# czbiohub-sf/shrimPy

Hardware: AMD Instinct MI355X
Metric: voxels/sec deskew+20-iter RL deconv, 2048×2048×512 f32; HBM GB/s vs peak (higher is better)
Workload: dtype f32

## Files before the change

shrimpy_amd/csrc/rl_fused_sep.hip:

```cpp

#include "common.hpp"
#include "correlate_common.hpp"

#ifndef LSR_FUSED_PZ
#error "compile with -DLSR_FUSED_PZ=<odd tap count along z>"
#endif

namespace {

using lsr::FusedArgs;

constexpr int kTX = lsr::kSepWideTileX;
constexpr int kWaves = 8;
constexpr int kThreads = 64 * kWaves;
constexpr int kBand = 8;
constexpr int kRing = 3;

constexpr int cdiv(int a, int b) { return (a + b - 1) / b; }

template <int PZ, int PYX, int RUN>
struct Geo {
  static constexpr int C = PYX / 2, CZ = PZ / 2;
  static constexpr int TY = 8 * RUN;
  static constexpr int WL = lsr::fused_window_halo(PYX);
  static constexpr int AR = TY + 4 * C;
  static constexpr int PA = kTX + 2 * WL;
  static constexpr int CH = PA / 4;
  static constexpr int NCH = AR * CH;
  static constexpr int SL = cdiv(NCH, kThreads);
  static constexpr int ASZ = cdiv(NCH, 64) * 64 * 4;
  static constexpr int NP = cdiv(4 + 2 * C, 4);
  static constexpr int G1 = (kTX + WL) / 4;
  static constexpr int PB1 = 4 * G1;
  static constexpr int NIT1 = AR * G1;
  static constexpr int XIT1 = cdiv(NIT1, kThreads);
  static constexpr int R1 = TY + 2 * C;
  static constexpr int RUN1 = cdiv(R1, 8);
  static constexpr int E = PB1 - kTX;
  static constexpr int NE = R1 * E;
  static constexpr int EP = cdiv(NE, kThreads);
  static constexpr int SH = WL - 2 * C;
  static constexpr int PR = 4 * (kTX / 4 - 1 + NP);
  static constexpr int RSZ = 4 + 8 * RUN1 * PR;
  static constexpr int NIT2 = R1 * (kTX / 4);
  static constexpr int XIT2 = cdiv(NIT2, kThreads);
  static constexpr int B1SZ = AR * PB1;
  static constexpr int B2SZ = R1 * kTX;
  static constexpr int OFF_B1 = kRing * ASZ;
  static constexpr int OFF_R = OFF_B1 + B1SZ;
  static constexpr int OFF_B2 = OFF_R + RSZ;
  static constexpr int OFF_DUMP = OFF_B2 + B2SZ;
  static constexpr int OFF_RNY = OFF_DUMP + 256;
  static constexpr int TOTAL = OFF_RNY + 32;
  static constexpr int NY = 2 * RUN1 + EP;
#ifdef LSR_FUSED_PROBE_NOXC
  static constexpr int NXC = 0;
#else
  static constexpr int NXC = 2 * RUN + 1;
#endif
  static_assert(TOTAL * 4 <= 160 * 1024, "LDS per workgroup");
  static_assert(PR == PB1, "B1 and R share a pitch");
  static_assert(2 * C <= WL && WL <= lsr::kSepOriginCol, "halo columns");
  static_assert(SL + 2 * (NY + NXC) <= 63, "vmcnt is a 6-bit counter");
  static_assert(OFF_B1 % 4 == 0 && OFF_R % 4 == 0 && OFF_B2 % 4 == 0, "16-byte aligned buffers");
};

typedef float f32x4 __attribute__((ext_vector_type(4)));
typedef float f32x2 __attribute__((ext_vector_type(2)));

__device__ __forceinline__ float fast_rcp(float d) {
  float r = __builtin_amdgcn_rcpf(d);
  return fmaf(fmaf(-d, r, 1.0f), r, r);
}
__device__ __forceinline__ f32x2 splat(float a) { return f32x2{a, a}; }
__device__ __forceinline__ f32x2 pk_fma(f32x2 a, f32x2 b, f32x2 c) { return __builtin_elementwise_fma(a, b, c); }
__device__ __forceinline__ f32x2 fast_rcp2(f32x2 d) {
  const f32x2 r = f32x2{__builtin_amdgcn_rcpf(d.x), __builtin_amdgcn_rcpf(d.y)};
  return pk_fma(pk_fma(-d, r, splat(1.0f)), r, r);
}
template <int PX, int NP>
__device__ __forceinline__ f32x4 xpass_item(const f32x4* src, const float (&wx)[PX]) {
  float w[4 * NP];
#pragma unroll
  for (int i = 0; i < NP; ++i) {
    const f32x4 v = src[i];
    w[4 * i] = v.x; w[4 * i + 1] = v.y; w[4 * i + 2] = v.z; w[4 * i + 3] = v.w;
  }
  f32x2 o01 = splat(wx[0]) * f32x2{w[0], w[1]};
  f32x2 o23 = splat(wx[0]) * f32x2{w[2], w[3]};
#pragma unroll
  for (int c = 1; c < PX; ++c) {
    o01 = pk_fma(splat(wx[c]), f32x2{w[c], w[c + 1]}, o01);
    o23 = pk_fma(splat(wx[c]), f32x2{w[c + 2], w[c + 3]}, o23);
  }
  return f32x4{o01.x, o01.y, o23.x, o23.y};
}

template <int IMM>
__device__ __forceinline__ void gload(float& dst, const float* sbase, int voff) {
  asm volatile("global_load_dword %0, %1, %2 offset:%3" : "+v"(dst) : "v"(voff), "s"(sbase), "n"(IMM) : "memory");
}
#ifndef LSR_FUSED_STORE_POLICY
#define LSR_FUSED_STORE_POLICY "nt"
#endif
#ifndef LSR_FUSED_GLDS_POLICY
#define LSR_FUSED_GLDS_POLICY ""
#endif
template <int IMM>
__device__ __forceinline__ void gstore(float* sbase, int voff, float v) {
  asm volatile("global_store_dword %0, %1, %2 offset:%3 " LSR_FUSED_STORE_POLICY
               :
               : "v"(voff), "v"(v), "s"(sbase), "n"(IMM)
               : "memory");
}
__device__ __forceinline__ void glds_x4(const float* sbase, int voff, unsigned lds_byte_addr) {
  asm volatile("s_mov_b32 m0, %2\n\ts_nop 0\n\tglobal_load_lds_dwordx4 %0, %1 " LSR_FUSED_GLDS_POLICY
               :
               : "v"(voff), "s"(sbase), "s"(lds_byte_addr)
               : "memory");
}
template <int N>
__device__ __forceinline__ void wait_vm() {
  asm volatile("s_waitcnt vmcnt(%0)" : : "n"(N) : "memory");
}
template <int K>
__device__ __forceinline__ void tie(float (&a)[K]) {
#pragma unroll
  for (int i = 0; i < K; ++i) asm volatile("" : "+v"(a[i]));
}
__device__ __forceinline__ void tie(float& a) { asm volatile("" : "+v"(a)); }
__device__ __forceinline__ void lds_barrier() {
  asm volatile("s_waitcnt lgkmcnt(0)" ::: "memory");
  __builtin_amdgcn_s_barrier();
  __builtin_amdgcn_sched_barrier(0);
}

template <int PZ, int PYX, int RUN, bool STATS>
__global__ __launch_bounds__(kThreads) void rl_fused_sep_kernel(FusedArgs p) {
  using T = Geo<PZ, PYX, RUN>;
  constexpr int C = T::C, CZ = T::CZ, TY = T::TY, RUN1 = T::RUN1, EP = T::EP;
  constexpr int NP = T::NP, NY = T::NY, NXC = T::NXC, SL = T::SL;
  __shared__ f32x4 smem4[T::TOTAL / 4];
  float* const smem = reinterpret_cast<float*>(smem4);
  f32x4* const B1_4 = smem4 + T::OFF_B1 / 4;
  const float* const B1 = smem + T::OFF_B1;
  float* const Rw = smem + T::OFF_R + 4;
  const f32x4* const R_4 = smem4 + T::OFF_R / 4 + 1;
  f32x4* const B2_4 = smem4 + T::OFF_B2 / 4;
  const float* const B2 = smem + T::OFF_B2;
  const unsigned lds_base =
      static_cast<unsigned>(reinterpret_cast<size_t>((__attribute__((address_space(3))) char*)smem4));

  const int tid = threadIdx.x;
  const int lane = tid & 63;
  const int wave = __builtin_amdgcn_readfirstlane(tid >> 6);

  auto xcd_contiguous = [](int b, int n) {
#ifdef LSR_FUSED_PLAIN_ORDER
    return b;
#endif
    const int per = n / 8, rem = n % 8;
    const int xcd = b % 8, idx = b / 8;
    return xcd * per + (xcd < rem ? xcd : rem) + idx;
  };
  const int Z = p.Z, Y = p.Y, X = p.X;
  int lin, zb, ze;
  if (static_cast<int>(blockIdx.x) < p.n_full) {
    lin = xcd_contiguous(blockIdx.x, p.n_full);
    zb = 0;
    ze = Z;
  } else {
    const int t = xcd_contiguous(blockIdx.x - p.n_full, gridDim.x - p.n_full);
    const int col = t / p.pieces;
    lin = p.n_full + col;
    zb = (t - col * p.pieces) * p.z_chunk;
    ze = min(zb + p.z_chunk, Z);
  }
  const int band = lin / (p.tiles_x * kBand);
  const int lb = lin - band * (p.tiles_x * kBand);
  const int band_h = min(kBand, p.tiles_y - band * kBand);
#if defined(LSR_FUSED_PLAIN_ORDER) && LSR_FUSED_PLAIN_ORDER == 2
  const int tx = lin % p.tiles_x;
  const int ty = lin / p.tiles_x;
  (void)lb; (void)band_h;
#else
  const int tx = lb / band_h;
  const int ty = band * kBand + (lb - tx * band_h);
#endif
  const int x0 = tx * kTX, y0 = ty * TY;
#ifdef LSR_FUSED_LAG
  if ((tx + ty) & 1) {
#pragma unroll
    for (int i = 0; i < LSR_FUSED_LAG; ++i) __builtin_amdgcn_s_sleep(127);
  }
#endif

  float tv0 = p.taps[lane], tv1 = p.taps[64 + (lane & 31)];
  auto load_taps = [&](int row, auto& w) {
#pragma unroll
    for (int i = 0; i < static_cast<int>(sizeof(w) / sizeof(float)); ++i) {
      const int f = row * 16 + i;
      w[i] = __int_as_float(__builtin_amdgcn_readlane(__float_as_int(f < 64 ? tv0 : tv1), f & 63));
    }
  };

  const float* const x_tile = p.x + (static_cast<int64_t>(y0 - 2 * C) * p.pitch + (x0 - T::WL));
  int s_voff[SL];
#pragma unroll
  for (int k = 0; k < SL; ++k) {
    const int e = min(tid + k * kThreads, T::NCH - 1);
    const int r = e / T::CH, c = e - r * T::CH;
    s_voff[k] = (r * p.pitch + 4 * c) * 4;
  }
  int a1_chunk[T::XIT1];
#pragma unroll
  for (int k = 0; k < T::XIT1; ++k) {
    const int i = min(tid + k * kThreads, T::NIT1 - 1);
    const int row = i / T::G1;
    a1_chunk[k] = i + row * (T::CH - T::G1);
  }
  const int r1_row0 = wave * RUN1;
  const int y1_col = r1_row0 * T::PB1 + lane;
  const int r_col = r1_row0 * T::PR + lane - T::SH;
  const bool interior = x0 - C >= 0 && x0 + kTX + C <= X && y0 - C >= 0 && y0 + TY + C <= Y;
  int e_b1[EP], e_voff[EP];
  int e_rc[EP];
#pragma unroll
  for (int e = 0; e < EP; ++e) {
    const int t = min(tid + e * kThreads, T::NE - 1);
    const int er = t / T::E, ec = t - er * T::E;
    e_b1[e] = er * T::PB1 + kTX + ec;
    e_rc[e] = (er << 16) | (kTX + ec);
    e_voff[e] = (er * p.y_pitch + kTX + ec) * 4;
  }
  const int y2_col = (wave * RUN) * kTX + lane;
  int xc_voff[RUN], o_voff[RUN], y_voff[RUN1];
#pragma unroll
  for (int m = 0; m < RUN; ++m) {
    xc_voff[m] = ((wave * RUN + m) * p.pitch + lane) * 4;
    o_voff[m] = ((wave * RUN + m) * p.out_pitch + lane) * 4;
  }
#pragma unroll
  for (int m = 0; m < RUN1; ++m) y_voff[m] = (min(r1_row0 + m, T::R1 - 1) * p.y_pitch + lane) * 4;
  float rnx[2];
#pragma unroll
  for (int cg = 0; cg < 2; ++cg) rnx[cg] = fast_rcp(p.nx[min(x0 + lane + 64 * cg, X - 1)]);
  float* const rny_lds = smem + T::OFF_RNY;
  if (tid < TY) rny_lds[tid] = fast_rcp(p.ny[min(y0 + tid, Y - 1)]);

  f32x2 acc1[PZ][RUN1], acc2[PZ][RUN];
  float acc1e[PZ][EP];
#pragma unroll
  for (int j = 0; j < PZ; ++j) {
#pragma unroll
    for (int i = 0; i < RUN1; ++i) acc1[j][i] = splat(0.0f);
#pragma unroll
    for (int i = 0; i < EP; ++i) acc1e[j][i] = 0.0f;
#pragma unroll
    for (int i = 0; i < RUN; ++i) acc2[j][i] = splat(0.0f);
  }
  float yv[2 * RUN1], ye[EP], xc[2 * RUN], nzv = 1.0f;
#pragma unroll
  for (int i = 0; i < 2 * RUN1; ++i) yv[i] = 0.0f;
#pragma unroll
  for (int i = 0; i < EP; ++i) ye[i] = 0.0f;
#pragma unroll
  for (int i = 0; i < 2 * RUN; ++i) xc[i] = 0.0f;
  const f32x2 rnx2 = f32x2{rnx[0], rnx[1]};
  f32x2 st_flux = splat(0.0f), st_total = splat(0.0f);
  float st_change = 0.0f;
  auto st_add = [&](f32x2 x_old, f32x2 xu, f32x2 v) {
    st_flux += xu;
    st_total += v;
    const f32x2 d = v - x_old;
    st_change += __builtin_fabsf(d.x);
    st_change += __builtin_fabsf(d.y);
  };
  __builtin_amdgcn_sched_barrier(0);

  auto clampz = [&](int z) { return min(max(z, 0), Z - 1); };
  auto issue_glds = [&](int plane, int slot) {
    const float* src = x_tile + static_cast<int64_t>(clampz(plane)) * p.plane;
    const unsigned dst = lds_base + (slot * T::ASZ + wave * 64 * 4) * 4;
#pragma unroll
    for (int k = 0; k < SL; ++k) {
      const bool live = wave * 64 + k * kThreads < T::NCH;
      glds_x4(src, s_voff[k], live ? dst + k * kThreads * 16 : lds_base + T::OFF_DUMP * 4);
    }
  };
  const float* const xc_tile = p.x + (static_cast<int64_t>(y0) * p.pitch + x0);
  const float* const y_tile = p.y + (static_cast<int64_t>(y0 - C) * p.y_pitch + (x0 + C - T::WL));
  float* const o_tile = p.out + (static_cast<int64_t>(y0) * p.out_pitch + x0);
  auto issue_xc = [&](int o) {
#ifdef LSR_FUSED_PROBE_NOXC
    return;
#endif
    const int oc = clampz(o);
    const float* base = xc_tile + static_cast<int64_t>(oc) * p.plane;
#pragma unroll
    for (int m = 0; m < RUN; ++m) {
      gload<0>(xc[m], base, xc_voff[m]);
      gload<256>(xc[RUN + m], base, xc_voff[m]);
    }
    gload<0>(nzv, p.nz + oc, 0);
  };
  auto issue_y = [&](int q) {
    const float* base = y_tile + static_cast<int64_t>(clampz(q)) * p.y_plane;
#pragma unroll
    for (int m = 0; m < RUN1; ++m) {
      gload<0>(yv[m], base, y_voff[m]);
      gload<256>(yv[RUN1 + m], base, y_voff[m]);
    }
#pragma unroll
    for (int e = 0; e < EP; ++e) gload<0>(ye[e], base, e_voff[e]);
  };

  const int q_lo = max(zb - CZ, 0), q_hi = min(ze - 1 + CZ, Z - 1);
  const int p_lo = max(q_lo - CZ, 0);
  const int p_hi = ze + 2 * CZ;

  int slot = 0;
  issue_glds(p_lo, 0);
  issue_xc(p_lo - 1 - 2 * CZ);
  issue_y(p_lo - CZ);
  issue_glds(p_lo + 1, 1);
  issue_xc(p_lo - 1 - 2 * CZ);
  issue_y(p_lo - CZ);
  wait_vm<SL + 2 * (NXC + NY)>();
  lds_barrier();

#ifdef LSR_FUSED_PROBE_TIME
  if (p.probe && tid == 0) p.probe[4 * blockIdx.x] = wall_clock64();
#endif
  for (int pz = p_lo; pz <= p_hi; ++pz) {
    asm volatile("" : "+v"(tv0), "+v"(tv1));
#ifdef LSR_FUSED_PROBE_TIME
    if (p.probe && tid == 0 && (pz == p_lo + 40 || pz == p_lo + 120))
      p.probe[4 * blockIdx.x + (pz == p_lo + 40 ? 1 : 2)] = wall_clock64();
#endif
    const int qr = pz - 1 - CZ;
    const int o = qr - CZ;
    const int q = pz - CZ;
    const bool x_live = pz < Z && pz <= q_hi + CZ;
    const bool r_live = qr >= q_lo && qr <= q_hi;
    const int slot2 = slot >= 1 ? slot - 1 : 2;

    issue_glds(pz + 2, slot2);
#ifdef LSR_FUSED_PROBE_NOCOMPUTE
    if (false) {
#else
    if (x_live) {
#endif
      float w1x[PYX];
      load_taps(0, w1x);
      const f32x4* A_4 = smem4 + slot * (T::ASZ / 4);
#pragma unroll
      for (int k = 0; k < T::XIT1; ++k)
        if (k + 1 < T::XIT1 || tid + k * kThreads < T::NIT1)
          B1_4[tid + k * kThreads] = xpass_item<PYX, NP>(A_4 + a1_chunk[k], w1x);
    } else {
#pragma unroll
      for (int k = 0; k < T::XIT1; ++k)
        if (k + 1 < T::XIT1 || tid + k * kThreads < T::NIT1) B1_4[tid + k * kThreads] = f32x4{0, 0, 0, 0};
    }
#ifdef LSR_FUSED_PROBE_NOCOMPUTE
    if (false) {
#else
    if (r_live) {
#endif
      float w2x[PYX];
      load_taps(3, w2x);
#pragma unroll
      for (int k = 0; k < T::XIT2; ++k) {
        const int j = tid + k * kThreads;
        if (k + 1 < T::XIT2 || j < T::NIT2)
          B2_4[j] = xpass_item<PYX, NP>(R_4 + (j + (j >> 5) * (T::PR / 4 - kTX / 4)), w2x);
      }
    } else {
#pragma unroll
      for (int k = 0; k < T::XIT2; ++k)
        if (k + 1 < T::XIT2 || tid + k * kThreads < T::NIT2) B2_4[tid + k * kThreads] = f32x4{0, 0, 0, 0};
    }
    lds_barrier();

    {
      float w2y[PYX], w2z[PZ];
      load_taps(4, w2y);
      load_taps(5, w2z);
      f32x2 pl[RUN];
#ifdef LSR_FUSED_PROBE_NOCOMPUTE
#pragma unroll
      for (int m = 0; m < RUN; ++m) pl[m] = splat(B2[y2_col + m]);
      if (false)
#endif
      {
        const float* colp = B2 + y2_col;
        f32x2 cv[RUN + 2 * C];
#pragma unroll
        for (int j = 0; j < RUN + 2 * C; ++j) cv[j] = f32x2{colp[j * kTX], colp[j * kTX + 64]};
#pragma unroll
        for (int m = 0; m < RUN; ++m) {
          f32x2 s2 = splat(w2y[0]) * cv[m];
#pragma unroll
          for (int b = 1; b < PYX; ++b) s2 = pk_fma(splat(w2y[b]), cv[m + b], s2);
          pl[m] = s2;
        }
      }
#pragma unroll
      for (int j = 0; j < PZ - 1; ++j)
#pragma unroll
        for (int i = 0; i < RUN; ++i) acc2[j][i] = pk_fma(splat(w2z[PZ - 1 - j]), pl[i], acc2[j + 1][i]);
#pragma unroll
      for (int i = 0; i < RUN; ++i) acc2[PZ - 1][i] = splat(w2z[0]) * pl[i];

      wait_vm<NY + SL>();
      tie(xc);
      tie(nzv);
#ifdef LSR_FUSED_PROBE_NOSTORE
      if (o >= zb && o < ze && nzv == 12345.678f) {
#else
      if (o >= zb && o < ze) {
#endif
        float* obase = o_tile + static_cast<int64_t>(o) * p.out_plane;
        const float rz = fast_rcp(nzv);
        if (!p.mask_out) {
#pragma unroll
          for (int m = 0; m < RUN; ++m) {
            const f32x2 xo = f32x2{xc[m], xc[RUN + m]};
            const f32x2 xu = xo * acc2[0][m];
            const f32x2 v = xu * (splat(rz * rny_lds[wave * RUN + m]) * rnx2);
            gstore<0>(obase, o_voff[m], v.x);
            gstore<256>(obase, o_voff[m], v.y);
            if constexpr (STATS) st_add(xo, xu, v);
          }
        } else {
          const bool ok0 = x0 + lane < X, ok1 = x0 + lane + 64 < X;
#pragma unroll
          for (int m = 0; m < RUN; ++m) {
            if (y0 + wave * RUN + m < Y) {
              const f32x2 xo = f32x2{xc[m], xc[RUN + m]};
              const f32x2 xu = xo * acc2[0][m];
              const f32x2 v = xu * (splat(rz * rny_lds[wave * RUN + m]) * rnx2);
              if (ok0) gstore<0>(obase, o_voff[m], v.x);
              if (ok1) gstore<256>(obase, o_voff[m], v.y);
              if constexpr (STATS) {
                st_add(xo, xu, v);
              }
            }
          }
        }
      }
      __builtin_amdgcn_sched_barrier(0);
      issue_xc(o + 1);
    }
    {
      float w1y[PYX], w1z[PZ];
      load_taps(1, w1y);
      load_taps(2, w1z);
      f32x2 pl[RUN1];
      float ple[EP];
#ifdef LSR_FUSED_PROBE_NOCOMPUTE
#pragma unroll
      for (int m = 0; m < RUN1; ++m) pl[m] = splat(B1[y1_col + m]);
      if (false)
#endif
      {
        const float* colp = B1 + y1_col;
        f32x2 cv[RUN1 + 2 * C];
#pragma unroll
        for (int j = 0; j < RUN1 + 2 * C; ++j) cv[j] = f32x2{colp[j * T::PB1], colp[j * T::PB1 + 64]};
#pragma unroll
        for (int m = 0; m < RUN1; ++m) {
          f32x2 s2 = splat(w1y[0]) * cv[m];
#pragma unroll
          for (int b = 1; b < PYX; ++b) s2 = pk_fma(splat(w1y[b]), cv[m + b], s2);
          pl[m] = s2;
        }
      }
#pragma unroll
      for (int e = 0; e < EP; ++e) {
        const float* colp = B1 + e_b1[e];
#ifdef LSR_FUSED_PROBE_NOCOMPUTE
        ple[e] = colp[0];
        continue;
#endif
        float s1 = w1y[0] * colp[0];
#pragma unroll
        for (int b = 1; b < PYX; ++b) s1 = fmaf(w1y[b], colp[b * T::PB1], s1);
        ple[e] = s1;
      }
#pragma unroll
      for (int j = 0; j < PZ - 1; ++j) {
#pragma unroll
        for (int i = 0; i < RUN1; ++i) acc1[j][i] = pk_fma(splat(w1z[PZ - 1 - j]), pl[i], acc1[j + 1][i]);
#pragma unroll
        for (int e = 0; e < EP; ++e) acc1e[j][e] = fmaf(w1z[PZ - 1 - j], ple[e], acc1e[j + 1][e]);
      }
#pragma unroll
      for (int i = 0; i < RUN1; ++i) acc1[PZ - 1][i] = splat(w1z[0]) * pl[i];
#pragma unroll
      for (int e = 0; e < EP; ++e) acc1e[PZ - 1][e] = w1z[0] * ple[e];

      wait_vm<SL + NXC>();
      tie(yv);
      tie(ye);
      const bool q_in = q >= q_lo && q <= q_hi;
      if (q_in && interior) {
#pragma unroll
        for (int m = 0; m < RUN1; ++m) {
          const f32x2 r = f32x2{yv[m], yv[RUN1 + m]} * fast_rcp2(acc1[0][m] + splat(p.eps));
          Rw[r_col + m * T::PR] = r.x;
          Rw[r_col + m * T::PR + 64] = r.y;
        }
#pragma unroll
        for (int e = 0; e < EP; ++e)
          if (e + 1 < EP || tid + e * kThreads < T::NE)
            Rw[e_b1[e] - T::SH] = ye[e] * fast_rcp(acc1e[0][e] + p.eps);
      } else {
        const int gx0 = x0 + lane + C - T::WL;
        const bool in0 = q_in && gx0 >= 0 && gx0 < X, in1 = q_in && gx0 + 64 >= 0 && gx0 + 64 < X;
#pragma unroll
        for (int m = 0; m < RUN1; ++m) {
          const int gy = y0 + r1_row0 + m - C;
          const bool row_in = gy >= 0 && gy < Y && r1_row0 + m < T::R1;
          const f32x2 r = f32x2{yv[m], yv[RUN1 + m]} * fast_rcp2(acc1[0][m] + splat(p.eps));
          Rw[r_col + m * T::PR] = (row_in && in0) ? r.x : 0.0f;
          Rw[r_col + m * T::PR + 64] = (row_in && in1) ? r.y : 0.0f;
        }
#pragma unroll
        for (int e = 0; e < EP; ++e) {
          if (e + 1 < EP || tid + e * kThreads < T::NE) {
            const int gy = y0 + (e_rc[e] >> 16) - C, gx = x0 + (e_rc[e] & 0xffff) + C - T::WL;
            const float r = ye[e] * fast_rcp(acc1e[0][e] + p.eps);
            Rw[e_b1[e] - T::SH] = (q_in && gy >= 0 && gy < Y && gx >= 0 && gx < X) ? r : 0.0f;
          }
        }
      }
      __builtin_amdgcn_sched_barrier(0);
      issue_y(q + 1);
    }
    wait_vm<SL + 2 * (NXC + NY)>();
    lds_barrier();
    slot = slot == 2 ? 0 : slot + 1;
  }
  asm volatile("s_waitcnt vmcnt(0)" ::: "memory");
  if constexpr (STATS) {
    lsr::keep_until_here(xc);
    lsr::keep_until_here(yv);
    lsr::keep_until_here(ye);
    lsr::keep_until_here(nzv);
    asm volatile("" : "+v"(st_flux), "+v"(st_total), "+v"(st_change));
    lsr::RlStats st;
    st.flux = st_flux.x + st_flux.y;
    st.change = st_change;
    st.total = st_total.x + st_total.y;
    lsr::rl_stats_flush<kWaves>(st, smem + T::OFF_B2, p.stats);
  }
#ifdef LSR_FUSED_PROBE_TIME
  if (p.probe && tid == 0) p.probe[4 * blockIdx.x + 3] = wall_clock64();
#endif
}

template <int PZ, int PYX>
bool launch_one(const FusedArgs& p, dim3 grid, hipStream_t s) {
  if constexpr (lsr::fused_compiled(PZ, PYX)) {
    constexpr int RUN = lsr::fused_run(PZ, PYX);
    if (p.stats != nullptr) hipLaunchKernelGGL((rl_fused_sep_kernel<PZ, PYX, RUN, true>), grid, dim3(kThreads), 0, s, p);
    else hipLaunchKernelGGL((rl_fused_sep_kernel<PZ, PYX, RUN, false>), grid, dim3(kThreads), 0, s, p);
    return true;
  } else {
    return false;
  }
}

}

namespace lsr {

#define LSR_CAT2(a, b) a##b
#define LSR_CAT(a, b) LSR_CAT2(a, b)
bool LSR_CAT(launch_fused_pz, LSR_FUSED_PZ)(int pyx, const FusedArgs& p, unsigned blocks, hipStream_t s) {
  constexpr int PZ = LSR_FUSED_PZ;
  const dim3 grid(blocks);
  switch (pyx) {
    case 3: return launch_one<PZ, 3>(p, grid, s);
    case 5: return launch_one<PZ, 5>(p, grid, s);
    case 7: return launch_one<PZ, 7>(p, grid, s);
    case 9: return launch_one<PZ, 9>(p, grid, s);
    case 11: return launch_one<PZ, 11>(p, grid, s);
    case 13: return launch_one<PZ, 13>(p, grid, s);
    case 15: return launch_one<PZ, 15>(p, grid, s);
    default: return false;
  }
}

}
```

Baseline: 40.46 billion.

## Keep delayed x planes in an LDS delay line instead of re-reading from HBM

```diff
diff --git a/shrimpy_amd/csrc/rl_fused_sep.hip b/shrimpy_amd/csrc/rl_fused_sep.hip
--- a/shrimpy_amd/csrc/rl_fused_sep.hip
+++ b/shrimpy_amd/csrc/rl_fused_sep.hip
@@ -14,9 +14,10 @@
 constexpr int kWaves = 8;
 constexpr int kThreads = 64 * kWaves;
 constexpr int kBand = 8;
-constexpr int kRing = 3;
+constexpr int kLdsFloats = 160 * 1024 / 4;
 
 constexpr int cdiv(int a, int b) { return (a + b - 1) / b; }
+constexpr int imin(int a, int b) { return a < b ? a : b; }
 
 template <int PZ, int PYX, int RUN>
 struct Geo {
@@ -46,23 +47,43 @@
   static constexpr int XIT2 = cdiv(NIT2, kThreads);
   static constexpr int B1SZ = AR * PB1;
   static constexpr int B2SZ = R1 * kTX;
-  static constexpr int OFF_B1 = kRing * ASZ;
+  static constexpr int D = PZ;
+  static constexpr int HXW = 8 * kTX * D;
+  static constexpr int FIXED = B1SZ + RSZ + B2SZ + 256 + 32;
+  static constexpr int hold_fit(int ring) {
+    return imin(RUN, (kLdsFloats - FIXED - ring * ASZ) / HXW);
+  }
+#ifdef LSR_FUSED_HOLD
+  static constexpr int HL = imin(LSR_FUSED_HOLD, hold_fit(2));
+#else
+  static constexpr int HL = hold_fit(3) > 0 ? hold_fit(3) : hold_fit(2);
+#endif
+#ifdef LSR_FUSED_RING
+  static constexpr int RING = LSR_FUSED_RING;
+#else
+  static constexpr int RING = HL <= hold_fit(3) ? 3 : 2;
+#endif
+  static constexpr int HOLD = 8 * HL;
+  static constexpr int OFF_B1 = RING * ASZ;
   static constexpr int OFF_R = OFF_B1 + B1SZ;
   static constexpr int OFF_B2 = OFF_R + RSZ;
   static constexpr int OFF_DUMP = OFF_B2 + B2SZ;
   static constexpr int OFF_RNY = OFF_DUMP + 256;
-  static constexpr int TOTAL = OFF_RNY + 32;
+  static constexpr int OFF_HX = OFF_RNY + 32;
+  static constexpr int TOTAL = OFF_HX + HL * HXW;
   static constexpr int NY = 2 * RUN1 + EP;
 #ifdef LSR_FUSED_PROBE_NOXC
   static constexpr int NXC = 0;
 #else
-  static constexpr int NXC = 2 * RUN + 1;
-#endif
+  static constexpr int NXC = 2 * (RUN - HL) + 1;
+#endif
+  static constexpr int VM_RING = (RING - 2) * SL + (RING - 1) * (NXC + NY);
   static_assert(TOTAL * 4 <= 160 * 1024, "LDS per workgroup");
   static_assert(PR == PB1, "B1 and R share a pitch");
   static_assert(2 * C <= WL && WL <= lsr::kSepOriginCol, "halo columns");
-  static_assert(SL + 2 * (NY + NXC) <= 63, "vmcnt is a 6-bit counter");
-  static_assert(OFF_B1 % 4 == 0 && OFF_R % 4 == 0 && OFF_B2 % 4 == 0, "16-byte aligned buffers");
+  static_assert(VM_RING <= 63 && SL + NY <= 63 && SL + NXC <= 63, "vmcnt is a 6-bit counter");
+  static_assert(OFF_B1 % 4 == 0 && OFF_R % 4 == 0 && OFF_B2 % 4 == 0 && OFF_HX % 4 == 0, "16-byte aligned buffers");
+  static_assert(0 <= HL && HL <= RUN && (RING == 3 || RING == 2), "delay line");
 };
 
 typedef float f32x4 __attribute__((ext_vector_type(4)));
@@ -139,7 +160,7 @@
 __global__ __launch_bounds__(kThreads) void rl_fused_sep_kernel(FusedArgs p) {
   using T = Geo<PZ, PYX, RUN>;
   constexpr int C = T::C, CZ = T::CZ, TY = T::TY, RUN1 = T::RUN1, EP = T::EP;
-  constexpr int NP = T::NP, NY = T::NY, NXC = T::NXC, SL = T::SL;
+  constexpr int NP = T::NP, NY = T::NY, NXC = T::NXC, SL = T::SL, HL = T::HL, RING = T::RING;
   __shared__ f32x4 smem4[T::TOTAL / 4];
   float* const smem = reinterpret_cast<float*>(smem4);
   f32x4* const B1_4 = smem4 + T::OFF_B1 / 4;
@@ -259,13 +280,15 @@
 #pragma unroll
     for (int i = 0; i < RUN; ++i) acc2[j][i] = splat(0.0f);
   }
-  float yv[2 * RUN1], ye[EP], xc[2 * RUN], nzv = 1.0f;
+  constexpr int NXR = RUN - HL;
+  constexpr int NXV = NXR > 0 ? 2 * NXR : 1;
+  float yv[2 * RUN1], ye[EP], xc[NXV], nzv = 1.0f;
 #pragma unroll
   for (int i = 0; i < 2 * RUN1; ++i) yv[i] = 0.0f;
 #pragma unroll
   for (int i = 0; i < EP; ++i) ye[i] = 0.0f;
 #pragma unroll
-  for (int i = 0; i < 2 * RUN; ++i) xc[i] = 0.0f;
+  for (int i = 0; i < NXV; ++i) xc[i] = 0.0f;
   const f32x2 rnx2 = f32x2{rnx[0], rnx[1]};
   f32x2 st_flux = splat(0.0f), st_total = splat(0.0f);
   float st_change = 0.0f;
@@ -298,9 +321,9 @@
     const int oc = clampz(o);
     const float* base = xc_tile + static_cast<int64_t>(oc) * p.plane;
 #pragma unroll
-    for (int m = 0; m < RUN; ++m) {
-      gload<0>(xc[m], base, xc_voff[m]);
-      gload<256>(xc[RUN + m], base, xc_voff[m]);
+    for (int m = HL; m < RUN; ++m) {
+      gload<0>(xc[m - HL], base, xc_voff[m]);
+      gload<256>(xc[NXR + m - HL], base, xc_voff[m]);
     }
     gload<0>(nzv, p.nz + oc, 0);
   };
@@ -320,13 +343,19 @@
   const int p_hi = ze + 2 * CZ;
 
   int slot = 0;
+  constexpr int HX_STEP = HL * kWaves * kTX;
+  int hx_i = T::OFF_HX + wave * kTX + lane;
+  int xa_i = (2 * C + wave * RUN) * T::PA + T::WL + lane;
+  if constexpr (HL > 0) asm volatile("" : "+v"(hx_i), "+v"(xa_i));
   issue_glds(p_lo, 0);
   issue_xc(p_lo - 1 - 2 * CZ);
   issue_y(p_lo - CZ);
-  issue_glds(p_lo + 1, 1);
-  issue_xc(p_lo - 1 - 2 * CZ);
-  issue_y(p_lo - CZ);
-  wait_vm<SL + 2 * (NXC + NY)>();
+  if constexpr (RING == 3) {
+    issue_glds(p_lo + 1, 1);
+    issue_xc(p_lo - 1 - 2 * CZ);
+    issue_y(p_lo - CZ);
+  }
+  wait_vm<T::VM_RING>();
   lds_barrier();
 
 #ifdef LSR_FUSED_PROBE_TIME
@@ -343,9 +372,9 @@
     const int q = pz - CZ;
     const bool x_live = pz < Z && pz <= q_hi + CZ;
     const bool r_live = qr >= q_lo && qr <= q_hi;
-    const int slot2 = slot >= 1 ? slot - 1 : 2;
-
-    issue_glds(pz + 2, slot2);
+    const int slot_in = slot >= 1 ? slot - 1 : RING - 1;
+
+    issue_glds(pz + RING - 1, slot_in);
 #ifdef LSR_FUSED_PROBE_NOCOMPUTE
     if (false) {
 #else
@@ -414,8 +443,14 @@
       for (int i = 0; i < RUN; ++i) acc2[PZ - 1][i] = splat(w2z[0]) * pl[i];
 
       wait_vm<NY + SL>();
-      tie(xc);
+#pragma unroll
+      for (int i = 0; i < 2 * NXR; ++i) tie(xc[i]);
       tie(nzv);
+      float* const hx = smem + hx_i;
+      auto x_out = [&](int m) -> f32x2 {
+        if (m < HL) return f32x2{hx[m * kWaves * kTX], hx[m * kWaves * kTX + 64]};
+        return f32x2{xc[m - HL], xc[NXR + m - HL]};
+      };
 #ifdef LSR_FUSED_PROBE_NOSTORE
       if (o >= zb && o < ze && nzv == 12345.678f) {
 #else
@@ -426,7 +461,7 @@
         if (!p.mask_out) {
 #pragma unroll
           for (int m = 0; m < RUN; ++m) {
-            const f32x2 xo = f32x2{xc[m], xc[RUN + m]};
+            const f32x2 xo = x_out(m);
             const f32x2 xu = xo * acc2[0][m];
             const f32x2 v = xu * (splat(rz * rny_lds[wave * RUN + m]) * rnx2);
             gstore<0>(obase, o_voff[m], v.x);
@@ -438,7 +473,7 @@
 #pragma unroll
           for (int m = 0; m < RUN; ++m) {
             if (y0 + wave * RUN + m < Y) {
-              const f32x2 xo = f32x2{xc[m], xc[RUN + m]};
+              const f32x2 xo = x_out(m);
               const f32x2 xu = xo * acc2[0][m];
               const f32x2 v = xu * (splat(rz * rny_lds[wave * RUN + m]) * rnx2);
               if (ok0) gstore<0>(obase, o_voff[m], v.x);
@@ -450,6 +485,15 @@
           }
         }
       }
+      if constexpr (HL > 0) {
+        const float* const a = smem + slot * T::ASZ + xa_i;
+#pragma unroll
+        for (int m = 0; m < HL; ++m) {
+          const float v0 = a[m * T::PA], v1 = a[m * T::PA + 64];
+          hx[m * kWaves * kTX] = v0;
+          hx[m * kWaves * kTX + 64] = v1;
+        }
+      }
       __builtin_amdgcn_sched_barrier(0);
       issue_xc(o + 1);
     }
@@ -539,13 +583,18 @@
       __builtin_amdgcn_sched_barrier(0);
       issue_y(q + 1);
     }
-    wait_vm<SL + 2 * (NXC + NY)>();
+    wait_vm<T::VM_RING>();
     lds_barrier();
-    slot = slot == 2 ? 0 : slot + 1;
+    slot = slot == RING - 1 ? 0 : slot + 1;
+    if constexpr (HL > 0) {
+      hx_i = hx_i + HX_STEP >= T::OFF_HX + T::D * HX_STEP ? hx_i + HX_STEP - T::D * HX_STEP : hx_i + HX_STEP;
+      asm volatile("" : "+v"(hx_i));
+    }
   }
   asm volatile("s_waitcnt vmcnt(0)" ::: "memory");
   if constexpr (STATS) {
-    lsr::keep_until_here(xc);
+#pragma unroll
+    for (int i = 0; i < 2 * NXR; ++i) lsr::keep_until_here(xc[i]);
     lsr::keep_until_here(yv);
     lsr::keep_until_here(ye);
     lsr::keep_until_here(nzv);
```

After: 40.41 billion, median of 3. No clear change (-0.1%).
